# yinwoods/k8s-scheduler

Hardware: AMD Instinct MI355X
Metric: pod-node evaluations/sec (higher is better)
Workload: dtype f64

## Files before the change

k8s-scheduler_amd/csrc/ksched_commit.h:

```cpp
#pragma once

#include <hip/hip_runtime.h>

#include <type_traits>

#ifndef KSCHED_XCHG_DEBUG
#define KSCHED_XCHG_DEBUG 0
#endif
#ifndef KSCHED_COMMIT_SPLIT
#define KSCHED_COMMIT_SPLIT 0
#endif

#include "ksched_pipe.h"

namespace ksched {

namespace {

constexpr int kSpcHashBits = 11;
constexpr int kSpcHash = 1 << kSpcHashBits;
template <bool LAG3>
constexpr int spc_slots() { return LAG3 ? 192 : 128; }
static_assert(spc_slots<true>() + 1 <= kRescueMaxT, "RescueReq::ti must hold the persistent commit's touched slots");
constexpr int kSpcInvalid = kSpcHash - 1;
constexpr int kGS = 14;
constexpr int kFoldMaskBytes = 16;

constexpr uint64_t kSkipKeyBits = 0x7ff8000000000badull;
__device__ __forceinline__ double skip_key() { return __longlong_as_double((long long)kSkipKeyBits); }
__device__ __forceinline__ float screen_y(int64_t a, double y) {
    return (a > 0 && a < (1ll << 52)) ? (float)y : __builtin_nanf("");
}

struct alignas(16) TouchY {
    float c, m, p, w;
};
__device__ __forceinline__ TouchY touch_stage(int64_t a0, int64_t a1, int64_t a2, double y0, double y1, double y2) {
    return TouchY{screen_y(a0, y0), screen_y(a1, y1), screen_y(a2, y2), 0.0f};
}
__device__ __forceinline__ bool touch_need(float qc, float qm, float qp, float thr, const TouchY &ty, int64_t rc, int64_t rm,
                                           int64_t rp, int64_t n0, int64_t n1, int64_t n2, bool active, float *v) {
    bool lo;
    *v = screen_pair(qc, qm, qp, ty.c, ty.m, ty.p, n0 >= rc, n1 >= rm, n2 >= rp, &lo);
    return active && !(*v < thr);
}
template <int PRIO, int DOM, bool F53>
__device__ __forceinline__ bool touch_column(float qc, float qm, float qp, float thr, const TouchY &ty, bool active,
// ... 435 lines not shown
        if (SCR)
            thr0 = (wave == 0 && pj) ? (int32_t)(uint32_t)(load_i64<COH>(
                                           reinterpret_cast<const int64_t *>(A.lists + (size_t)lane * K + 1) + 6) >> 32) : 0;
#pragma unroll
        for (int u = 0; u < kHeadPer; ++u) {
            const int e = tid + u * kSpcThreads;
            w0[u] = 0; w1[u] = 0;
            if (e < 64 * K && e / K < nb) {
                const uint64_t *w = reinterpret_cast<const uint64_t *>(A.lists + e);
                if (COH) { w0[u] = ld_coh(w); w1[u] = ld_coh(w + 1); }
                else { w0[u] = w[0]; w1[u] = w[1]; }
            }
        }
    };
    if constexpr (!COH) load_lists();

    int n1 = 0, n2 = 0, nin = 0;
    uint64_t dbg_x1 = 0;
    (void)dbg_x1;
    const double rcf = (double)rc, rmf = (double)rm, rpf = (double)rp;
    const double y3 = recip(3.0);
    double *Srow = m.S + (size_t)lane * kSpcRow;
    uint64_t smv[3] = {0, 0, 0};
    auto key_inherited = [&](int ne, auto sl) {
        int dfl = 0;
        double pk = -__builtin_inf();
        int32_t pi = kNoIdx, ps = -1;
        const float thrf = SCR ? m.thr[lane] : 0.0f;
        const float qc = screen_req(rc), qm = screen_req(rm), qp = screen_req(rp);
        int64_t nex = 0;
        int tv = 0;
        if constexpr (SCR) {
            const int ev = wave + lane * kSpcWaves;
            tv = ev < ne ? sl(ev) : 0;
        }
        for (int e = wave, u = 0; e < ne; e += kSpcWaves, ++u) {
            const int t = SCR ? __builtin_amdgcn_readlane(tv, u) : sl(e);
            const SpcSlot &x = m.T[t];
            const int64_t *x0 = m.s0 + e * 3;
            const bool f0 = fits(rc, rm, rp, sel, x0[0], x0[1], x0[2], x.labels, LAB);
            const bool f1 = fits(rc, rm, rp, sel, x.cur[0], x.cur[1], x.cur[2], x.labels, LAB);
            dfl += (int)f1 - (int)f0;
            const double *yy = m.iy + e * 6;
            double k;
            if constexpr (SCR) {
                const bool any = touch_column<PRIO, DOM, F53>(qc, qm, qp, thrf, m.iyt[e], pj, f1, rc, rm, rp, rcf, rmf, rpf,
                                                              x.cur[0], x.cur[1], x.cur[2], yy, y3, x.price, &k);
                Srow[t] = k;
                if (!any) continue;
                ++nex;
            } else {
                ++nex;
                const bool el = pair_key_fast<PRIO, DOM, F53>(f1, rc, rm, rp, rcf, rmf, rpf, x.cur[0], x.cur[1], x.cur[2],
                                                              yy[0], yy[1], yy[2], yy[3], yy[4], yy[5], y3, x.price, &k);
                k = el ? k : -__builtin_inf();
                Srow[t] = k;
            }
            const bool up = k != -__builtin_inf() && better(k, x.idx, pk, pi);
            pk = up ? k : pk; pi = up ? x.idx : pi; ps = up ? t : ps;
        }
        if constexpr (SCR) {
            if (nex > 0 || A.fold_all) {
                m.pbk[wave * 64 + lane] = pk;
                m.pbx[wave * 64 + lane] = ((int64_t)ps << 32) | (uint32_t)pi;
                if (lane == 0) atomicOr(&m.fm[3], 1u << wave);
            }
        } else {
            m.pbk[wave * 64 + lane] = pk;
            m.pbx[wave * 64 + lane] = ((int64_t)ps << 32) | (uint32_t)pi;
        }
        if (dfl != 0) atomicAdd(&m.dfacc[lane], dfl);
        if (SCR && A.dbg && lane == 0 && wave < ne) {
            atomicAdd(reinterpret_cast<unsigned long long *>(&A.dbg[16]), (unsigned long long)((ne - 1 - wave) / kSpcWaves + 1));
            atomicAdd(reinterpret_cast<unsigned long long *>(&A.dbg[17]), (unsigned long long)nex);
        }
    };
    auto hash_lists = [&]() {
#pragma unroll
        for (int u = 0; u < kHeadPer; ++u) {
            const int e = tid + u * kSpcThreads;
            if (e < 64 * K) {
                const int j = e / K, q = e % K;
                const bool v = (uint32_t)(w1[u] >> 32) != 0;
                const double key = v ? __longlong_as_double((long long)w0[u]) : -__builtin_inf();
                const int32_t idx = v ? (int32_t)(uint32_t)w1[u] : kNoIdx;
                m.LK[q * 64 + j] = key;
                m.LI[q * 64 + j] = idx;
                m.HP[q * 64 + j] = idx == kNoIdx ? kSpcInvalid : spc_pos_insert(m.hk, idx);
            }
        }
    };
    if constexpr (!COH) {
        n1 = A.xin->count;
        XRec xi{};
        if (wave == 0 && lane < n1) xi = load_xrec<COH>(A.xin->e, lane);
        for (int w = tid; w < kSpcHash; w += kSpcThreads) m.hk[w] = -1;
// ... 144 lines not shown
                SpcSlot &x = m.T[slot];
                x.idx = xi.idx; x.mine = 0;
                for (int r = 0; r < 3; ++r) { m.s0[lane * 3 + r] = xi.sb[r]; x.sb[r] = xi.cur[r]; x.cur[r] = xi.cur[r]; }
                x.labels = xi.labels; x.price = xi.price; x.pad = 0;
                m.ti[slot] = xi.idx;
                m.gs[lane] = slot;
                if constexpr (SCR) {
                    double st[6];
                    stage_state(st, xi.cur);
#pragma unroll
                    for (int r = 0; r < 6; ++r) m.iy[lane * 6 + r] = st[r];
                    m.iyt[lane] = touch_stage(xi.cur[0], xi.cur[1], xi.cur[2], st[3], st[4], st[5]);
                } else {
                    stage_state(m.iy + lane * 6, xi.cur);
                }
                if (dup) m.x2s[slot] = -1;
                else atomicOr(&m.tkc[h >> 5], 1u << (h & 31));
            }
            if (lane == 0) m.ctl[3] = n2 + __popcll(nm);
        }
        __syncthreads();
        if (tid == 0 && A.trace_row) A.trace_row[23] = wall_clock64();
        nin = m.ctl[3];
        key_inherited(n1, [&](int e) { return (int)m.gs[e]; });
        __syncthreads();
        if (tid == 0 && A.trace_row) A.trace_row[24] = wall_clock64();
    }

    int32_t fcc = 0;
    double rbk = -__builtin_inf();
    int32_t rbi = kNoIdx, rbs = -1;
    constexpr bool RB2 = COH && PRIO == kPrioResource && DOM == kDomAll;
    bool trk = false;
    int cv = 0, cut = 0;
    int32_t my_idx = 0, my_feas = 0;
    int32_t my_src = 0;
    double my_score = 0.0;
    int32_t my_g = -2, my_q = -1, my_s = -1, my_h = kSpcInvalid;
    int nT = nin, done = nb, W = 64;
    int nresc = 0;
    int rcredit = 0, rmax = 0;
    if constexpr (COH) {
        const int c = A.loc->rescue_credit + A.rescue_rate;
        rcredit = c < 4 * A.rescue_cap ? c : 4 * A.rescue_cap;
        rmax = rcredit >= 2 * A.rescue_cap ? A.rescue_max : A.rescue_low;
    }
    int64_t placed = 0, nrounds = 0, nfail = 0, niters = 0, nseq = 0;
    int nfull = 0;
    static_assert(kSpcWaves <= 32, "SpcSmem::fm: a wave mask is one 32-bit word");
    constexpr uint32_t kAllWaves = 0xffffffffu >> (32 - kSpcWaves);
    auto fm_count = [&](int w, int64_t v) {
        if (v) atomicAdd(reinterpret_cast<unsigned long long *>(&A.dbg[w]), (unsigned long long)v);
    };
    if (wave == 0) {
        int64_t ds2 = 0;
        double xk = -__builtin_inf();
        int32_t xix = kNoIdx, xe = -1;
        if (LAG3 && A.batch >= 2 && n2 > 0 && pj) {
            ds2 = (int64_t)smv[0];
            xk = __longlong_as_double((long long)smv[1]);
            xix = (int32_t)(uint32_t)smv[2];
            xe = (int32_t)(smv[2] >> 32);
        }
        fcc = pj ? (int32_t)(fc0v + m.dfacc[lane] + ds2) : 0;
        cut = cut0;
#pragma unroll
        for (int q = 0; q < K; ++q) cv += m.LI[q * 64 + lane] != kNoIdx;
        if constexpr (SCR) {
            uint32_t wm = (uint32_t)__builtin_amdgcn_readfirstlane((int)m.fm[3]) | (A.fold_all & kAllWaves);
            if (dbg && lane == 0) {
                fm_count(34, wm == 0);
                m.ctl[3] = 0;
            }
            for (; wm != 0; wm &= wm - 1u) {
                const int w = __builtin_ctz(wm);
                const double k = m.pbk[w * 64 + lane];
                const int64_t x = m.pbx[w * 64 + lane];
                const int32_t xi = (int32_t)(uint32_t)x;
                if (k != -__builtin_inf() && better(k, xi, rbk, rbi)) { rbk = k; rbi = xi; rbs = (int32_t)(x >> 32); }
            }
        } else {
            for (int w = 0; w < kSpcWaves; ++w) {
                const double k = m.pbk[w * 64 + lane];
                const int64_t x = m.pbx[w * 64 + lane];
                const int32_t xi = (int32_t)(uint32_t)x;
                if (k != -__builtin_inf() && better(k, xi, rbk, rbi)) { rbk = k; rbi = xi; rbs = (int32_t)(x >> 32); }
            }
        }
        if (LAG3 && xix != kNoIdx) {
            if (m.x2s[xe] >= 0) {
                if (better(xk, xix, rbk, rbi)) { rbk = xk; rbi = xix; rbs = m.x2s[xe]; }
            } else {
                for (int e = 0; e < n2; ++e) {
                    if (m.x2s[e] < 0) continue;
                    const double k = Srow[m.x2s[e]];
                    const int32_t xi = m.ti[m.x2s[e]];
                    if (k != -__builtin_inf() && better(k, xi, rbk, rbi)) { rbk = k; rbi = xi; rbs = m.x2s[e]; }
                }
            }
        }
        if (lane == 0) { m.ctl[0] = 0; m.ctl[2] = 0; }
    }

    auto rekey_row = [&](int f, double &wk, int32_t &wi, int &s) {
        const int64_t fc = rl64(rc, f), fm = rl64(rm, f), fp = rl64(rp, f);
        const uint64_t fs = (uint64_t)rl64((int64_t)sel, f);
        const double fcf = (double)fc, fmf = (double)fm, fpf = (double)fp;
        double *row = m.S + (size_t)f * kSpcRow;
        int64_t nrk = 0;
        for (int t0 = 0; t0 < nT; t0 += 64) {
            const int t = t0 + lane;
            double k = -__builtin_inf();
            int32_t x = kNoIdx, ts_ = t;
            if (t < nT && row[t] != row[t]) {
                const SpcSlot &y = m.T[t];
                const bool fy = fits(fc, fm, fp, fs, y.cur[0], y.cur[1], y.cur[2], y.labels, LAB);
                k = lane_key<PRIO, DOM, LAB, F53>(fy, fc, fm, fp, fcf, fmf, fpf, y.cur[0], y.cur[1], y.cur[2], y3, y.price);
                row[t] = k;
                x = k != -__builtin_inf() ? y.idx : kNoIdx;
                ++nrk;
            }
            wave_argbest_fast(k, x, ts_);
            if (x != kNoIdx && better(k, x, wk, wi)) { wk = k; wi = x; s = ts_; }
        }
// ... 20 lines not shown
                const bool u1 = v[u + 1] != -__builtin_inf() && better(v[u + 1], x[u + 1], k1, i1);
                if constexpr (T2) { const double o1 = u1 ? k1 : v[u + 1]; q1 = o1 > q1 ? o1 : q1; }
                if (u1) { k1 = v[u + 1]; i1 = x[u + 1]; s1 = t + u + 1; }
            }
        }
        for (; t < nT; ++t) {
            const double v = Srow[t];
            const int32_t x = m.ti[t];
            const bool u0 = v != -__builtin_inf() && better(v, x, k0, i0);
            if constexpr (T2) { const double o0 = u0 ? k0 : v; q0 = o0 > q0 ? o0 : q0; }
            if (u0) { k0 = v; i0 = x; s0 = t; }
        }
        q0 = q1 > q0 ? q1 : q0;
        if (k1 != -__builtin_inf() && better(k1, i1, k0, i0)) {
            q0 = k0 > q0 ? k0 : q0;
            k0 = k1; i0 = i1; s0 = s1;
        } else {
            q0 = k1 > q0 ? k1 : q0;
        }
        rbk = k0; rbi = i0; rbs = s0;
        if constexpr (T2) m.rb2[lane] = __double2float_ru(q0);
    };
    int c = 0;
    if (COH && tid == 0 && A.trace_row) A.trace_row[25] = wall_clock64();
    uint64_t *const tr1 = (COH && tid == 0) ? A.trace_row : nullptr;
    bool first = true;
    const uint64_t t_pro = dbg ? __builtin_amdgcn_s_memtime() - t_start : 0;
    for (;;) {
        if (dbg) t_mark = __builtin_amdgcn_s_memtime();
        if (wave == 0) {
            const int cend = (c + W < nb) ? c + W : nb;
            lds_order();
            for (int w = lane * 4; w < kSpcHash; w += 256) *reinterpret_cast<int4 *>(m.own + w) = make_int4(64, 64, 64, 64);
            lds_order();
            const uint64_t fitm = __ballot(fcc != 0);
            const bool act = lane >= c && lane < cend && ((fitm >> lane) & 1);
            constexpr int G = K < 8 ? K : 8;
            const uint32_t hp_at = lds_addr(m.HP + lane), own_at = lds_addr(m.own);
            uint32_t am = 0;
#pragma unroll
            for (int g = 0; g < K; g += G) {
                int32_t hp[G], tw[G];
                lds_gather<G, 5>(hp_at + g * 256, lds_addr(m.tkc), hp, tw);
#pragma unroll
                for (int u = 0; u < G; ++u) am |= (((uint32_t)tw[u] >> (hp[u] & 31)) & 1u) ? 0u : (1u << (g + u));
            }
            if (!act) am = 0;
            const uint32_t am1 = am & (am - 1u), amr = am1 & (am1 - 1u);
            const int32_t q0 = am ? (int32_t)__builtin_ctz(am) : 0, q1 = am1 ? (int32_t)__builtin_ctz(am1) : 0;
            int32_t h0, h1;
            lds_read2(hp_at + q0 * 256, hp_at + q1 * 256, h0, h1);
            int32_t pq = -1, ph = kSpcInvalid;
            for (int it = 0;; ++it) {
                ++niters;
                int32_t nq, nh;
                {
                    int32_t o0, o1;
                    lds_read2(own_at + h0 * 4, own_at + h1 * 4, o0, o1);
                    const bool ok0 = am != 0u && o0 >= lane, ok1 = am1 != 0u && o1 >= lane;
                    nq = ok0 ? q0 : (ok1 ? q1 : -1);
                    nh = ok0 ? h0 : (ok1 ? h1 : kSpcInvalid);
                    if (__ballot(amr != 0u && !ok0 && !ok1) != 0) {
                        ++nfull;
                        nq = -1; nh = kSpcInvalid;
#pragma unroll
                        for (int g = K - G; g >= 0; g -= G) {
                            int32_t hp[G], ow[G];
                            lds_gather<G, 0>(hp_at + g * 256, own_at, hp, ow);
#pragma unroll
// ... 2 lines not shown
                                nq = ok ? g + u : nq;
                                nh = ok ? hp[u] : nh;
                            }
                        }
                    }
                }
                const bool changed = __ballot(act && nq != pq) != 0;
                if (act && pq >= 0) m.own[ph] = 64;
                lds_order();
                pq = nq; ph = nh;
                if (!changed && it > 0) break;
                if (act && pq >= 0) atomicMin(&m.own[ph], lane);
                lds_order();
            }
            const uint64_t gm = __ballot(act && pq >= 0);
            if (lane >= c && lane < cend) {
                my_g = act ? (pq >= 0 ? 0 : -1) : -2;
                my_q = pq;
                my_h = act && pq >= 0 ? ph : kSpcInvalid;
                my_s = act && pq >= 0 ? nT + lanes_below(gm) : -1;
            }
            const bool in = lane >= c && lane < cend;
            if (in && my_g == 0) my_g = m.LI[my_q * 64 + lane];
            m.gn[lane] = in ? my_g : -2;
            m.gq[lane] = my_q;
            m.gs[lane] = my_s;
            m.fcg[lane] = 0;
            if constexpr (SCR) {
                if (lane < 3) m.fm[lane] = 0;
            }
            if (lane == 0) { m.ctl[0] = c; m.ctl[1] = cend; }
        }
        __syncthreads();
        if (first && tr1) tr1[49] = wall_clock64();
        if (dbg) { const uint64_t t = __builtin_amdgcn_s_memtime(); t_s1 += t - t_mark; t_mark = t; }
        const int rc0 = m.ctl[0], rce = m.ctl[1];
        {
            double pk = -__builtin_inf();
            int32_t pi = kNoIdx, ps = -1;
            if (wave == 0 && lane >= rc0 && lane < rce && m.gn[lane] >= 0) {
                const uint64_t *src = reinterpret_cast<const uint64_t *>(A.lists + (size_t)lane * K + m.gq[lane]) + 2;
                uint64_t v[5];
#pragma unroll
                for (int w = 0; w < 5; ++w) v[w] = COH ? ld_coh(src + w) : src[w];
                const int64_t n0 = wsub((int64_t)v[0], rc), n1 = wsub((int64_t)v[1], rm), n2 = wsub((int64_t)v[2], 1);
                const double nf0 = (double)n0, nf1 = (double)n1, nf2 = (double)n2;
                uint64_t *o = m.GS + (size_t)lane * kGS;
                if constexpr (SCR) {
                    const double ny0 = recip_or_zero(n0, nf0), ny1 = recip_or_zero(n1, nf1), ny2 = recip_or_zero(n2, nf2);
                    SpcSlot &x = m.T[my_s];
                    x.idx = my_g; x.mine = 1;
                    x.sb[0] = (int64_t)v[0]; x.sb[1] = (int64_t)v[1]; x.sb[2] = (int64_t)v[2];
                    x.cur[0] = n0; x.cur[1] = n1; x.cur[2] = n2;
                    x.labels = v[3]; x.price = __uint_as_float((uint32_t)v[4]); x.pad = 0;
                    m.ti[my_s] = my_g;
                    *reinterpret_cast<TouchY *>(o) = touch_stage(n0, n1, n2, ny0, ny1, ny2);
                    o[8] = (uint64_t)__double_as_longlong(nf0); o[9] = (uint64_t)__double_as_longlong(nf1);
                    o[10] = (uint64_t)__double_as_longlong(nf2);
                    o[11] = (uint64_t)__double_as_longlong(ny0);
// ... 578 lines not shown
```

k8s-scheduler_amd/csrc/ksched_ctx.h:

```cpp
#pragma once

#include <hip/hip_runtime.h>
#include <rccl/rccl.h>

#include <algorithm>
#include <chrono>
#include <condition_variable>
#include <cstdint>
#include <memory>
#include <mutex>
#include <optional>
#include <string>
#include <vector>

#include "ksched.h"
#include "ksched_exact.h"
#include "ksched_kernels.h"
#include "ksched_pipe.h"
#include "ksched_stream.h"

struct ksched_group {
    int nranks = 0, dev = 0;
    int64_t block_bytes = 0;
    std::vector<const char *> send;
// ... 77 lines not shown
    DevBuf<int32_t> bprio, btidx, bdepth, bseg;
    DevBuf<void> vws;
    DevBuf<void> pws;
    DevBuf<uint64_t> trace;
    DevBuf<uint64_t> trace_wg;
    DevBuf<uint64_t> xdbg;
    DevBuf<int32_t> xmin;
};

struct ksched_diag {
    bool trace = false;
    std::string trace_dump;
    std::string trace_wg;
    std::string xchg_dump;
    bool commit_stamps = false;
    bool merge_stamps = false;
    bool debug = false;
    bool no_screen = false;
    bool no_pairs = false;
    bool no_seed = false;
    bool touch_screen = true;
    bool no_fold_mask = false;
    bool early_inh = true;
    bool poison = false;
    std::optional<uint32_t> lds_fill;
    int lds_role = 7;
    int lds_lo = 0;
    std::optional<int> lds_hi;
    uint32_t jitter = 0;
    bool plain_launch = false;
    int exact1_bs = 1024;
    int xchg_diag = 0;
    int64_t epoch_base = 0;
    int64_t persist_timeout_ms = 10000;
    int64_t exchange_timeout_ms = 2000;
    int rescue_max = 4;
    int rescue_rate = 4;
    int rescue_cap = 16;
    int rescue_low = 2;
    int rescue_look = 0;
};

struct ksched_ctx {
    ksched_opts o{};
    int dev = 0;
    int cus = 256;
// ... 122 lines not shown
```

k8s-scheduler_amd/csrc/ksched_diag.hip:

```cpp
#include <cstdio>
#include <cstdlib>
#include <cstring>

#include "ksched_ctx.h"

namespace ksched {

static int env_int(const char *name, int dflt) {
    const char *v = std::getenv(name);
    return v && *v ? std::atoi(v) : dflt;
}
static std::string env_str(const char *name) {
    const char *v = std::getenv(name);
    return v ? v : "";
}

void read_env(ksched_diag *d) {
    d->trace = env_int("KSCHED_PERSIST_TRACE", 0) != 0;
    d->trace_dump = env_str("KSCHED_TRACE_DUMP");
    d->trace_wg = env_str("KSCHED_TRACE_WG");
    d->xchg_dump = env_str("KSCHED_XCHG_DUMP");
    d->commit_stamps = env_int("KSCHED_COMMIT_STAMPS", 0) != 0;
    d->merge_stamps = env_int("KSCHED_MERGE_STAMPS", 0) != 0;
    d->debug = env_int("KSCHED_DEBUG", 0) != 0;
    d->no_screen = env_int("KSCHED_NO_SCREEN", 0) != 0;
    d->no_pairs = env_int("KSCHED_NO_PAIRS", 0) != 0;
    d->no_seed = env_int("KSCHED_NO_SEED", 0) != 0;
    d->touch_screen = env_int("KSCHED_NO_TOUCH_SCREEN", 0) == 0;
    d->no_fold_mask = env_int("KSCHED_NO_FOLD_MASK", 0) != 0;
    d->early_inh = env_int("KSCHED_NO_EARLY_INH", 0) == 0;
    d->poison = env_int("KSCHED_POISON", 0) != 0;
    if (const std::string f = env_str("KSCHED_LDS_FILL"); !f.empty()) d->lds_fill = (uint32_t)std::strtoul(f.c_str(), nullptr, 0);
    d->lds_role = env_int("KSCHED_LDS_ROLE", 7);
    d->lds_lo = env_int("KSCHED_LDS_LO", 0);
    if (!env_str("KSCHED_LDS_HI").empty()) d->lds_hi = env_int("KSCHED_LDS_HI", 0);
    d->jitter = (uint32_t)env_int("KSCHED_JITTER", 0);
    d->plain_launch = env_int("KSCHED_PLAIN_LAUNCH", 0) != 0;
    d->exact1_bs = env_int("KSCHED_EXACT1_BS", 1024);
    d->xchg_diag = env_int("KSCHED_XCHG_DIAG", 0);
    d->epoch_base = env_int("KSCHED_XCHG_EPOCH_BASE", 0);
    d->persist_timeout_ms = env_int("KSCHED_PERSIST_TIMEOUT_MS", 10000);
    d->exchange_timeout_ms = env_int("KSCHED_EXCHANGE_TIMEOUT_MS", 2000);
    d->rescue_max = env_int("KSCHED_RESCUE_MAX", 4);
    d->rescue_rate = env_int("KSCHED_RESCUE_RATE", 4);
    d->rescue_cap = env_int("KSCHED_RESCUE_CAP", 16);
    d->rescue_low = env_int("KSCHED_RESCUE_LOW", 2);
    d->rescue_look = env_int("KSCHED_RESCUE_LOOK", 0);
}

static void write_u64(const std::string &path, const int64_t *hdr, size_t nhdr, const std::vector<uint64_t> &t) {
    if (FILE *f = std::fopen(path.c_str(), "wb")) {
        if (nhdr) std::fwrite(hdr, 8, nhdr, f);
        std::fwrite(t.data(), 8, t.size(), f);
// ... 53 lines not shown
                    "exactly %.4f | sequential columns %lld, exactly %.4f | rescue re-keys %lld\n", (long long)hd[16],
                    (double)hd[17] / std::max<int64_t>(1, hd[16]), (long long)hd[18], (double)hd[19] / std::max<int64_t>(1, hd[18]),
                    (long long)hd[20], (double)hd[21] / std::max<int64_t>(1, hd[20]), (long long)hd[22]);
        if (hd[14])
            fprintf(stderr, "persist commit guess: iterations %lld, of them past the two lowest entries (all K scanned) %lld | "
                    "pods resolved one by one %lld\n", (long long)hd[5], (long long)hd[8], (long long)hd[31]);
        if (hd[14])
            fprintf(stderr, "persist commit: batches=%lld rounds/batch %.3f guess iterations/round %.2f failures %lld | "
                    "cycles/batch: before the wait %.0f (other waves %.0f) entry to past the wait %.0f (poll %.0f, poll + barrier %.0f, early read sufficed %.3f, early inh read sufficed %lld of %lld) | prologue %.0f guess %.0f evaluate %.0f check %.0f total %.0f\n",
                    (long long)hd[14], (double)hd[12] / hd[14], (double)hd[5] / std::max<int64_t>(1, hd[12]),
                    (long long)hd[13], (double)hd[6] / hd[14], (double)hd[9] / hd[14] / 11.0, (double)hd[7] / hd[14], (double)hd[10] / hd[14], (double)hd[11] / hd[14], (double)hd[15] / hd[14], (long long)hd[29], (long long)hd[30], (double)hd[0] / hd[14],
                    (double)hd[1] / hd[14], (double)hd[2] / hd[14], (double)hd[3] / hd[14], (double)hd[4] / hd[14]);
        if (hd[14])
            fprintf(stderr, "persist commit rescans: steps with a worsened holder %lld, every holder kept %lld | plain rescans "
                    "%lld, %.0f cycles each | with the second-best key %lld, %.0f cycles each\n", (long long)hd[23],
                    (long long)hd[24], (long long)hd[25], (double)hd[26] / std::max<int64_t>(1, hd[25]), (long long)hd[27],
                    (double)hd[28] / std::max<int64_t>(1, hd[27]));
        if (hd[14] && hd[16])
            fprintf(stderr, "persist commit fold masks: checks that read no partials %lld of %lld, partial rows read %lld | "
                    "wave-0 states that read none %lld of %lld | confirm-fold columns visited %lld skipped %lld | batches "
                    "with a check that read none after one that read some %lld\n", (long long)hd[32], (long long)hd[12],
                    (long long)hd[33], (long long)hd[34], (long long)hd[14], (long long)hd[35], (long long)hd[36],
                    (long long)hd[37]);
    }
    if (c->d->mdbg) {
        int64_t hm[8];
        if (hipMemcpy(hm, c->d->mdbg, sizeof(hm), hipMemcpyDeviceToHost) == hipSuccess && hm[7]) {
            const double nwg = (double)hm[7];
            fprintf(stderr, "persist merge: merges=%lld | cycles/merge: loads %.0f rank-heads %.0f barrier %.0f "
                    "global-heads %.0f rank-entries %.0f write %.0f\n", (long long)hm[7], hm[0] / nwg, hm[1] / nwg,
                    hm[2] / nwg, hm[3] / nwg, hm[4] / nwg, hm[5] / nwg);
        }
    }
    if (!cnt) return;
    const double us = 0.01 / (double)cnt;
    fprintf(stderr,
            "persist trace: %lld batches, period %.2f us | to-score %.2f score %.2f merge %.2f to-commit %.2f "
            "commit %.2f commit-gap %.2f (to loop top %.2f, top to past the wait %.2f) | wg0: poll %.2f apply %.2f "
            "score %.2f (rows %.2f slowest-wave %.2f fold %.2f stores %.2f) | merger poll %.2f\n",
            (long long)cnt, 0.01 * (double)(int64_t)(at(last, 4) - at(first, 4)) / (double)std::max<int64_t>(1, last - first),
            sum[0] * us, sum[1] * us, sum[2] * us, sum[3] * us, sum[4] * us, sum[5] * us, sum[14] * us, sum[15] * us, sum[6] * us, sum[7] * us,
            sum[8] * us, sum[10] * us, sum[11] * us, sum[12] * us, sum[13] * us, sum[9] * us);
    if (nscr)
        fprintf(stderr, "persist screen (WG 0 wave 0): %lld of %lld batches screened | pass 1 / seed pass %.2f us, other waves "
                "%.2f us, bound %.2f us, pass 2 / single pass %.2f us, exact phase %.2f us (%.2f of the workgroup's %d rows needed; pair lists in %lld batches, "
                "%.1f pairs each)\n", (long long)nscr, (long long)cnt,
// ... 189 lines not shown
```

k8s-scheduler_amd/csrc/ksched_engine.hip:

```cpp
#include <cmath>
#include <cstdio>
#include <cstring>

#include "ksched_ctx.h"
#include "ksched_why.h"

using namespace ksched;

namespace {

hipError_t ev_take(ksched_ctx *c, int *idx) {
    if (c->ev_used >= c->ev_pool.size()) {
        hipEvent_t e;
        hipError_t r = hipEventCreate(&e);
        if (r != hipSuccess) return r;
        c->ev_pool.push_back(e);
    }
    *idx = (int)c->ev_used++;
    return hipSuccess;
}

hipError_t ev_begin(ksched_ctx *c, bool on, int *e0, hipStream_t s) {
    if (!on) return hipSuccess;
    hipError_t r = ev_take(c, e0);
// ... 242 lines not shown
    const size_t inh_b = align_up(inh_bytes(B), 256);
    const size_t need = part_b + 4 * lists_b + 5 * xb + prog_b + resc_b + inh_b;
    if (c->d->pws.bytes < need) c->d_prog = nullptr;
    HIPCHK(c, c->d->pws.reserve(need));
    char *w = static_cast<char *>(c->d->pws.p);
    a.nodes = c->d->nodes; a.n_local = n;
    a.pods = PodArgs{c->d->rc, c->d->rm, c->d->rp, c->d->sel, c->p};
    a.ctl = reinterpret_cast<Ctl *>(c->d->cursor.p);
    a.part = reinterpret_cast<Cand *>(w);
    a.lring = w + part_b;
    a.lists_bytes = (int64_t)lists_b;
    a.xring = a.lring + 4 * lists_b;
    a.xbuf_bytes = (int64_t)xb;
    a.prog = reinterpret_cast<uint64_t *>(a.xring + 5 * xb);
    a.rescue = c->diag.rescue_max <= 0 ? nullptr : reinterpret_cast<char *>(a.prog) + prog_b;
    a.rescue_max = c->diag.rescue_max;
    a.rescue_rate = c->diag.rescue_rate;
    a.rescue_look = c->diag.rescue_look;
    a.rescue_cap = c->diag.rescue_cap;
    a.rescue_low = c->diag.rescue_low;
    a.touch_screen = c->diag.touch_screen ? 1 : 0;
    a.early_inh = c->diag.early_inh ? 1 : 0;
    a.no_fold_mask = c->diag.no_fold_mask ? 1 : 0;
    if (c->diag.jitter) a.jitter = c->diag.jitter * 2654435761u + (uint32_t)(++c->jitter_calls) * 40503u + 1u;
    a.inh = reinterpret_cast<char *>(a.prog) + prog_b + resc_b;
    c->d_prog = a.prog;
    c->prog_G = G;
    c->prog_rows = R;
    c->prog_B = B;
    a.out = OutArgs{c->d->oidx, c->d->osc, c->d->ofeas};
    fill_xchg_args(c, &a);
    a.err = c->d->err;
    a.timeout_ticks = c->diag.persist_timeout_ms * 100000;
    a.no_screen = c->diag.no_screen ? 1 : 0;
    a.no_pairs = c->diag.no_pairs ? 1 : 0;
    a.no_seed = c->diag.no_seed ? 1 : 0;
    if (c->diag.trace) {
        const int64_t cap = 4 * (c->p / B) + 64;
        HIPCHK(c, c->d->trace.reserve((size_t)cap * kTraceCols * 8));
        HIPCHK(c, hipMemsetAsync(c->d->trace, 0, c->d->trace.bytes, c->stream));
        a.trace = c->d->trace;
        a.trace_cap = c->trace_rows();
    }
    if (!c->diag.trace_wg.empty()) {
        const int64_t elems = (4 * (c->p / B) + 64) * (int64_t)G;
        HIPCHK(c, c->d->trace_wg.reserve((size_t)elems * 8));
// ... 450 lines not shown
```

k8s-scheduler_amd/csrc/ksched_kernels.h:

```cpp
#pragma once

#include "ksched_device.h"

namespace ksched {

struct alignas(16) XRec {
    int32_t idx;
    int32_t pad;
    int64_t cur[3];
    int64_t sb[3];
    uint64_t labels;
    float price;
    int32_t pad2;
    int64_t pad3;
};
static_assert(sizeof(XRec) == 80, "XRec layout");

template <bool COH>
__device__ __forceinline__ void add_i64(int64_t *p, int64_t v) {
    if (COH) st_coh(p, (uint64_t)((int64_t)ld_coh(p) + v)); else *p += v;
}

struct alignas(16) XBuf {
    int32_t count;
// ... 57 lines not shown
constexpr int kRecWords = (int)(sizeof(Rec) / 4);
constexpr int msg_words(int K) { return K * kRecWords + 2; }

struct PersistArgs;
struct PersistLocal;
struct CommitArgs {
    const Rec *lists;
    const int64_t *fc0;
    PodArgs pods;
    const int64_t *plan;
    const int64_t *plan1;
    int64_t *plan2;
    Ctl *ctl;
    int32_t B;
    const XBuf *xin;
    const XBuf *xin2;
    XBuf *xout;
    OutArgs out;
    int64_t *dbg;
    int64_t batch;
    int64_t *cursor_at;
    PersistLocal *loc;
    int32_t release;
    char *rescue;
    int32_t rescue_n;
    int32_t rescue_max;
    int32_t rescue_cap;
    int32_t rescue_low;
    int32_t rescue_look;
    int32_t rescue_rate;
    int32_t touch_screen;
    uint32_t fold_all;
    const char *inh;
    int64_t timeout_ticks;
    int32_t *err;
    uint64_t *trace_row;
    const PersistArgs *xp;
    int64_t dbg_act;
};
constexpr int kCommitDbgWords = 48;
constexpr int kSpcThreads = 512;

template <bool COH = false>
__device__ __forceinline__ void publish_committed(const CommitArgs &A) {
    if (!COH) {
        if ((threadIdx.x & 63) == 0 && A.cursor_at) st_coh(A.cursor_at, ld_coh(&A.ctl->cursor));
// ... 119 lines not shown
```

k8s-scheduler_amd/csrc/ksched_pipe.h:

```cpp
#pragma once

#include "ksched_kernels.h"

namespace ksched {

constexpr uint32_t kXRecPipe = 96;
constexpr size_t xbuf_bytes_pipe(int B) { return 16 + (size_t)2 * B * kXRecPipe; }
__device__ __forceinline__ int64_t w64(uint32_t lo, uint32_t hi) { return (int64_t)(((uint64_t)hi << 32) | lo); }

__device__ __forceinline__ bool load_xrec_pipe(const XRec *e, int i, uint32_t tag, XRec *o) {
    const __amdgpu_buffer_rsrc_t r = coh_rsrc(e);
    const uint32_t off = (uint32_t)i * kXRecPipe;
    u32x4 c[6];
#pragma unroll
    for (int k = 0; k < 6; ++k) c[k] = ld_coh16(r, off + 16u * k);
    o->idx = (int32_t)c[0].y; o->pad = 0;
    o->cur[0] = w64(c[0].z, c[0].w); o->cur[1] = w64(c[1].y, c[1].z); o->cur[2] = w64(c[1].w, c[2].y);
    o->sb[0] = w64(c[2].z, c[2].w); o->sb[1] = w64(c[3].y, c[3].z); o->sb[2] = w64(c[3].w, c[4].y);
    o->labels = (uint64_t)w64(c[4].z, c[4].w);
    o->price = __uint_as_float(c[5].y); o->pad2 = 0; o->pad3 = 0;
    return (c[0].x == tag) & (c[1].x == tag) & (c[2].x == tag) & (c[3].x == tag) & (c[4].x == tag) & (c[5].x == tag);
}

template <bool COH>
// ... 90 lines not shown
    int64_t *mdbg;
    int64_t node_offset;
    int32_t R, rank;
    uint32_t epoch0;
    int64_t xchg_stride;
    char *rx_peer[8];
    uint64_t *prog;
    char *rescue;
    int32_t poison_lds;
    uint32_t lds_fill;
    int32_t lds_fill_role;
    int32_t lds_fill_lo, lds_fill_hi;
    uint32_t jitter;
    int32_t rescue_max;
    int32_t rescue_cap;
    int32_t rescue_low;
    int32_t rescue_look;
    int32_t rescue_rate;
    int32_t touch_screen;
    char *inh;
    int32_t early_inh;
    int32_t no_seed;
    int32_t no_fold_mask;
};
constexpr size_t inh_bytes(int B) { return (size_t)4 * B * 32 + (size_t)4 * B * 64 * 8; }
constexpr int kProgWords = 6;
constexpr int kSeedWords = 2;
__host__ __device__ inline size_t prog_seed_off(int G, int B, int commit_wgs) { return (size_t)(G + B + commit_wgs) * kProgWords; }
enum : int { kProgWaitCommit = 1, kProgScan = 2, kProgArrived = 3, kProgWaitArrive = 4, kProgMerged = 5,
             kProgWaitMerged = 6, kProgCommitted = 7, kProgIdle = 8, kProgRescue = 9, kProgWaitRescue = 10,
             kProgTimedOut = 0x80 };
__device__ __forceinline__ uint32_t hw_where() {
    uint32_t xcc, hw;
    asm volatile("s_getreg_b32 %0, hwreg(HW_REG_XCC_ID)" : "=s"(xcc));
    asm volatile("s_getreg_b32 %0, hwreg(HW_REG_HW_ID)" : "=s"(hw));
    return (xcc & 0xf) << 8 | ((hw >> 13) & 7) << 4 | ((hw >> 8) & 0xf);
}
__device__ __forceinline__ void prog_at(const PersistArgs &P, int slot, int64_t b, int phase, uint64_t seen) {
    if (!P.prog) return;
    __hip_atomic_store(P.prog + kProgWords * slot, (uint64_t)b << 8 | (uint64_t)phase, __ATOMIC_RELAXED,
                       __HIP_MEMORY_SCOPE_AGENT);
    __hip_atomic_store(P.prog + kProgWords * slot + 1, (uint64_t)hw_where() << 32 | (seen & 0xffffffffull),
                       __ATOMIC_RELAXED, __HIP_MEMORY_SCOPE_AGENT);
}
__device__ __forceinline__ void prog_add(const PersistArgs &P, int slot, uint64_t scan, uint64_t busy) {
    if (!P.prog || !P.trace) return;
// ... 168 lines not shown
```

k8s-scheduler_amd/csrc/ksched_pipe.hip:

```cpp
#include <hip/hip_fp16.h>
#include <hip/hip_runtime.h>

#include <cstdio>
#include <cstdlib>

#include "ksched_commit.h"
#include "ksched_merge.h"

#ifndef KSCHED_PIPE_PART
#define KSCHED_PIPE_PART 0
#endif

namespace ksched {

namespace {

constexpr int kSW = kPipeScoreWaves;
constexpr int kMT = kPipeMergeThreads;
constexpr int kMW = kMT / 64;
constexpr int kMS = kPipeMergeSlots;
constexpr int kPU = 4;
#ifndef KSCHED_XCHG_DEBUG
#define KSCHED_XCHG_DEBUG 0
#endif
// ... 1448 lines not shown
        ca.plan = &ctl->plan[b % kPlanRing];
        ca.plan1 = &ctl->plan[(b + kPipeLag - 1) % kPlanRing];
        ca.plan2 = &ctl->plan[(b + kPipeLag) % kPlanRing];
        ca.xin = reinterpret_cast<const XBuf *>(P.xring + (size_t)(b >= 1 ? (b - 1) % 4 : 4) * P.xbuf_bytes);
        ca.xin2 = reinterpret_cast<const XBuf *>(P.xring + (size_t)(b >= 2 ? (b - 2) % 4 : 4) * P.xbuf_bytes);
        ca.xout = reinterpret_cast<XBuf *>(P.xring + (size_t)(b % 4) * P.xbuf_bytes);
        ca.out = P.out;
        ca.batch = b;
        ca.cursor_at = &ctl->cursor_at[b % kPlanRing];
        ca.dbg = P.cdbg;
        ca.trace_row = (P.trace && b < P.trace_cap) ? P.trace + b * kTraceCols : nullptr;
        ca.loc = &loc;
        ca.rescue = P.rescue;
        ca.xp = &P;
        ca.dbg_act = nact - 1;
        ca.rescue_n = P.B;
        ca.rescue_max = P.rescue_max;
        ca.rescue_rate = P.rescue_rate;
        ca.rescue_look = P.rescue_look;
        ca.rescue_cap = P.rescue_cap;
        ca.rescue_low = P.rescue_low;
        ca.touch_screen = P.touch_screen;
        ca.fold_all = P.no_fold_mask ? ~0u : 0u;
        ca.inh = P.inh;
        ca.timeout_ticks = P.timeout_ticks;
        ca.err = P.err;
        const int rc = commit_spc_batch<K, PRIO, DOM, LAB, F53, true, kPipeThreads>(ca, cs, &pre, wait_merged, handoff, inh_ready);
        if (rc == 2) return;
        if (rc == 0) {
            if (threadIdx.x == 0) atomicCAS(P.err, 0, kErrWaitMerged);
            if (threadIdx.x < 64) publish_committed_all(ctl, 1ull << 62);
            return;
        }
        __syncthreads();
        if (threadIdx.x < kCanaryBytes / 4 && canary[threadIdx.x] != (0xA5A5A5A5u ^ threadIdx.x)) {
            if (atomicCAS(P.err, 0, kErrLdsCanary) == 0 && P.prog)
                P.prog[kProgWords * cslot + 2] = (uint64_t)b << 32 | (uint64_t)threadIdx.x << 16 | (canary[threadIdx.x] & 0xffffu);
        }
        if (threadIdx.x == 0) {
            trace_at(P, b, 4);
            prog_at(P, cslot, b, kProgCommitted, 0);
        }
        if (loc.cursor >= P.pods.p) {
            if (threadIdx.x < 64) publish_committed_all(ctl, 1ull << 62);
            return;
        }
// ... 153 lines not shown
```

Baseline: 313.6 billion.

## Overlap wave 0's first guess round with inherited key scoring in persistent commit

In the persistent (coherent) commit path, wave 0 now starts the first guess/ownership round while the other waves compute inherited keys, instead of waiting behind a barrier. Wave 0's share of key scoring is spread over the remaining waves, and each wave's per-lane best is held in registers until after the barrier. The guess is redone only if the true fit mask differs from the one it assumed. This takes key scoring off the critical path before the first round, at the cost of extra control flow, an occasional wasted guess and more register pressure. The behaviour is controlled by an environment flag and is on by default.

```diff
diff --git a/k8s-scheduler_amd/csrc/ksched_commit.h b/k8s-scheduler_amd/csrc/ksched_commit.h
--- a/k8s-scheduler_amd/csrc/ksched_commit.h
+++ b/k8s-scheduler_amd/csrc/ksched_commit.h
@@ -23,6 +23,8 @@
 constexpr int spc_slots() { return LAG3 ? 192 : 128; }
 static_assert(spc_slots<true>() + 1 <= kRescueMaxT, "RescueReq::ti must hold the persistent commit's touched slots");
 constexpr int kSpcInvalid = kSpcHash - 1;
+static_assert(kSpcInvalid >= 0 && kSpcInvalid < kSpcHash && (kSpcHash & (kSpcHash - 1)) == 0,
+              "kSpcInvalid: a position inside the table, which spc_pos_insert's probe sequence skips");
 constexpr int kGS = 14;
 constexpr int kFoldMaskBytes = 16;
 
@@ -504,7 +506,13 @@
     const double y3 = recip(3.0);
     double *Srow = m.S + (size_t)lane * kSpcRow;
     uint64_t smv[3] = {0, 0, 0};
+    [[maybe_unused]] bool early_keys = false;
+    double kp_k = -__builtin_inf();
+    int64_t kp_x = 0;
+    bool kp_w = false;
     auto key_inherited = [&](int ne, auto sl) {
+        const bool defer = COH && early_keys;
+        const int kw = defer ? wave - 1 : wave, ks = defer ? kSpcWaves - 1 : kSpcWaves;
         int dfl = 0;
         double pk = -__builtin_inf();
         int32_t pi = kNoIdx, ps = -1;
@@ -513,10 +521,10 @@
         int64_t nex = 0;
         int tv = 0;
         if constexpr (SCR) {
-            const int ev = wave + lane * kSpcWaves;
+            const int ev = kw + lane * ks;
             tv = ev < ne ? sl(ev) : 0;
         }
-        for (int e = wave, u = 0; e < ne; e += kSpcWaves, ++u) {
+        for (int e = kw, u = 0; e < ne; e += ks, ++u) {
             const int t = SCR ? __builtin_amdgcn_readlane(tv, u) : sl(e);
             const SpcSlot &x = m.T[t];
             const int64_t *x0 = m.s0 + e * 3;
@@ -543,17 +551,23 @@
         }
         if constexpr (SCR) {
             if (nex > 0 || A.fold_all) {
-                m.pbk[wave * 64 + lane] = pk;
-                m.pbx[wave * 64 + lane] = ((int64_t)ps << 32) | (uint32_t)pi;
+                if (COH && defer) {
+                    kp_k = pk; kp_x = ((int64_t)ps << 32) | (uint32_t)pi; kp_w = true;
+                } else {
+                    m.pbk[wave * 64 + lane] = pk;
+                    m.pbx[wave * 64 + lane] = ((int64_t)ps << 32) | (uint32_t)pi;
+                }
                 if (lane == 0) atomicOr(&m.fm[3], 1u << wave);
             }
+        } else if (COH && defer) {
+            kp_k = pk; kp_x = ((int64_t)ps << 32) | (uint32_t)pi; kp_w = true;
         } else {
             m.pbk[wave * 64 + lane] = pk;
             m.pbx[wave * 64 + lane] = ((int64_t)ps << 32) | (uint32_t)pi;
         }
         if (dfl != 0) atomicAdd(&m.dfacc[lane], dfl);
-        if (SCR && A.dbg && lane == 0 && wave < ne) {
-            atomicAdd(reinterpret_cast<unsigned long long *>(&A.dbg[16]), (unsigned long long)((ne - 1 - wave) / kSpcWaves + 1));
+        if (SCR && A.dbg && lane == 0 && kw < ne) {
+            atomicAdd(reinterpret_cast<unsigned long long *>(&A.dbg[16]), (unsigned long long)((ne - 1 - kw) / ks + 1));
             atomicAdd(reinterpret_cast<unsigned long long *>(&A.dbg[17]), (unsigned long long)nex);
         }
     };
@@ -744,10 +758,8 @@
         __syncthreads();
         if (tid == 0 && A.trace_row) A.trace_row[23] = wall_clock64();
         nin = m.ctl[3];
-        key_inherited(n1, [&](int e) { return (int)m.gs[e]; });
-        __syncthreads();
-        if (tid == 0 && A.trace_row) A.trace_row[24] = wall_clock64();
-    }
+    }
+    [[maybe_unused]] const bool early = COH && A.early_guess != 0;
 
     int32_t fcc = 0;
     double rbk = -__builtin_inf();
@@ -774,54 +786,47 @@
     auto fm_count = [&](int w, int64_t v) {
         if (v) atomicAdd(reinterpret_cast<unsigned long long *>(&A.dbg[w]), (unsigned long long)v);
     };
-    if (wave == 0) {
-        int64_t ds2 = 0;
-        double xk = -__builtin_inf();
-        int32_t xix = kNoIdx, xe = -1;
-        if (LAG3 && A.batch >= 2 && n2 > 0 && pj) {
-            ds2 = (int64_t)smv[0];
-            xk = __longlong_as_double((long long)smv[1]);
-            xix = (int32_t)(uint32_t)smv[2];
-            xe = (int32_t)(smv[2] >> 32);
-        }
-        fcc = pj ? (int32_t)(fc0v + m.dfacc[lane] + ds2) : 0;
-        cut = cut0;
-#pragma unroll
-        for (int q = 0; q < K; ++q) cv += m.LI[q * 64 + lane] != kNoIdx;
-        if constexpr (SCR) {
-            uint32_t wm = (uint32_t)__builtin_amdgcn_readfirstlane((int)m.fm[3]) | (A.fold_all & kAllWaves);
-            if (dbg && lane == 0) {
-                fm_count(34, wm == 0);
-                m.ctl[3] = 0;
-            }
-            for (; wm != 0; wm &= wm - 1u) {
-                const int w = __builtin_ctz(wm);
-                const double k = m.pbk[w * 64 + lane];
-                const int64_t x = m.pbx[w * 64 + lane];
-                const int32_t xi = (int32_t)(uint32_t)x;
-                if (k != -__builtin_inf() && better(k, xi, rbk, rbi)) { rbk = k; rbi = xi; rbs = (int32_t)(x >> 32); }
-            }
-        } else {
+    if constexpr (!COH) {
+        if (wave == 0) {
+            fcc = pj ? (int32_t)(fc0v + m.dfacc[lane]) : 0;
+            cut = cut0;
+#pragma unroll
+            for (int q = 0; q < K; ++q) cv += m.LI[q * 64 + lane] != kNoIdx;
             for (int w = 0; w < kSpcWaves; ++w) {
                 const double k = m.pbk[w * 64 + lane];
                 const int64_t x = m.pbx[w * 64 + lane];
                 const int32_t xi = (int32_t)(uint32_t)x;
                 if (k != -__builtin_inf() && better(k, xi, rbk, rbi)) { rbk = k; rbi = xi; rbs = (int32_t)(x >> 32); }
             }
-        }
-        if (LAG3 && xix != kNoIdx) {
-            if (m.x2s[xe] >= 0) {
-                if (better(xk, xix, rbk, rbi)) { rbk = xk; rbi = xix; rbs = m.x2s[xe]; }
-            } else {
-                for (int e = 0; e < n2; ++e) {
-                    if (m.x2s[e] < 0) continue;
-                    const double k = Srow[m.x2s[e]];
-                    const int32_t xi = m.ti[m.x2s[e]];
-                    if (k != -__builtin_inf() && better(k, xi, rbk, rbi)) { rbk = k; rbi = xi; rbs = m.x2s[e]; }
-                }
-            }
-        }
-        if (lane == 0) { m.ctl[0] = 0; m.ctl[2] = 0; }
+            if (lane == 0) { m.ctl[0] = 0; m.ctl[2] = 0; }
+        }
+    } else {
+        if (wave == 0) {
+            int64_t ds2 = 0;
+            double xk = -__builtin_inf();
+            int32_t xix = kNoIdx, xe = -1;
+            if (A.batch >= 2 && n2 > 0 && pj) {
+                ds2 = (int64_t)smv[0];
+                xk = __longlong_as_double((long long)smv[1]);
+                xix = (int32_t)(uint32_t)smv[2];
+                xe = (int32_t)(smv[2] >> 32);
+            }
+            fcc = pj ? (int32_t)(fc0v + ds2) : 0;
+            cut = cut0;
+            if (xix != kNoIdx) {
+                if (m.x2s[xe] >= 0) {
+                    if (better(xk, xix, rbk, rbi)) { rbk = xk; rbi = xix; rbs = m.x2s[xe]; }
+                } else {
+                    for (int e = 0; e < n2; ++e) {
+                        if (m.x2s[e] < 0) continue;
+                        const double k = Srow[m.x2s[e]];
+                        const int32_t xi = m.ti[m.x2s[e]];
+                        if (k != -__builtin_inf() && better(k, xi, rbk, rbi)) { rbk = k; rbi = xi; rbs = m.x2s[e]; }
+                    }
+                }
+            }
+            if (lane == 0) { m.ctl[0] = 0; m.ctl[2] = 0; }
+        }
     }
 
     auto rekey_row = [&](int f, double &wk, int32_t &wi, int &s) {
@@ -888,29 +893,41 @@
         if constexpr (T2) m.rb2[lane] = __double2float_ru(q0);
     };
     int c = 0;
-    if (COH && tid == 0 && A.trace_row) A.trace_row[25] = wall_clock64();
     uint64_t *const tr1 = (COH && tid == 0) ? A.trace_row : nullptr;
     bool first = true;
     const uint64_t t_pro = dbg ? __builtin_amdgcn_s_memtime() - t_start : 0;
+    [[maybe_unused]] uint64_t fitp = 0;
     for (;;) {
         if (dbg) t_mark = __builtin_amdgcn_s_memtime();
+        [[maybe_unused]] bool g = true, st = true;
+        [[maybe_unused]] bool more = false, skip_bar = false;
+        if constexpr (COH) { g = !first || early; st = !first; }
+#pragma nounroll
+        do {
         if (wave == 0) {
             const int cend = (c + W < nb) ? c + W : nb;
+            if (!COH || g) {
             lds_order();
             for (int w = lane * 4; w < kSpcHash; w += 256) *reinterpret_cast<int4 *>(m.own + w) = make_int4(64, 64, 64, 64);
             lds_order();
             const uint64_t fitm = __ballot(fcc != 0);
+            if constexpr (COH) fitp = fitm;
             const bool act = lane >= c && lane < cend && ((fitm >> lane) & 1);
             constexpr int G = K < 8 ? K : 8;
             const uint32_t hp_at = lds_addr(m.HP + lane), own_at = lds_addr(m.own);
             uint32_t am = 0;
+            [[maybe_unused]] int cvn = 0;
 #pragma unroll
             for (int g = 0; g < K; g += G) {
                 int32_t hp[G], tw[G];
                 lds_gather<G, 5>(hp_at + g * 256, lds_addr(m.tkc), hp, tw);
 #pragma unroll
-                for (int u = 0; u < G; ++u) am |= (((uint32_t)tw[u] >> (hp[u] & 31)) & 1u) ? 0u : (1u << (g + u));
-            }
+                for (int u = 0; u < G; ++u) {
+                    am |= (((uint32_t)tw[u] >> (hp[u] & 31)) & 1u) ? 0u : (1u << (g + u));
+                    if constexpr (COH) cvn += hp[u] != kSpcInvalid;
+                }
+            }
+            if constexpr (COH) cv = cvn;
             if (!act) am = 0;
             const uint32_t am1 = am & (am - 1u), amr = am1 & (am1 - 1u);
             const int32_t q0 = am ? (int32_t)__builtin_ctz(am) : 0, q1 = am1 ? (int32_t)__builtin_ctz(am1) : 0;
@@ -959,6 +976,9 @@
             }
             const bool in = lane >= c && lane < cend;
             if (in && my_g == 0) my_g = m.LI[my_q * 64 + lane];
+            }
+            if (!COH || st) {
+            const bool in = lane >= c && lane < cend;
             m.gn[lane] = in ? my_g : -2;
             m.gq[lane] = my_q;
             m.gs[lane] = my_s;
@@ -967,11 +987,67 @@
                 if (lane < 3) m.fm[lane] = 0;
             }
             if (lane == 0) { m.ctl[0] = c; m.ctl[1] = cend; }
-        }
-        __syncthreads();
+            }
+        }
+        if constexpr (COH) {
+            more = first && !st;
+            if (more) {
+                early_keys = early;
+                kp_w = false;
+                if (wave != 0 || !early) key_inherited(n1, [&](int e) { return (int)m.gs[e]; });
+                __syncthreads();
+                if (tr1) tr1[24] = wall_clock64();
+                if (early) {
+                    bool anyp = true;
+                    if constexpr (SCR) anyp = ((uint32_t)m.fm[3] | A.fold_all) != 0;
+                    if (kp_w) {
+                        m.pbk[wave * 64 + lane] = kp_k;
+                        m.pbx[wave * 64 + lane] = kp_x;
+                    }
+                    if (anyp) __syncthreads();
+                }
+                if (wave == 0) {
+                    fcc = pj ? fcc + m.dfacc[lane] : 0;
+                    if constexpr (SCR) {
+                        uint32_t wm = (uint32_t)__builtin_amdgcn_readfirstlane((int)m.fm[3]) |
+                                      (A.fold_all & kAllWaves & (early ? ~1u : ~0u));
+                        if (dbg && lane == 0) {
+                            fm_count(34, wm == 0);
+                            m.ctl[3] = 0;
+                        }
+                        for (; wm != 0; wm &= wm - 1u) {
+                            const int w = __builtin_ctz(wm);
+                            const double k = m.pbk[w * 64 + lane];
+                            const int64_t x = m.pbx[w * 64 + lane];
+                            const int32_t xi = (int32_t)(uint32_t)x;
+                            if (k != -__builtin_inf() && better(k, xi, rbk, rbi)) { rbk = k; rbi = xi; rbs = (int32_t)(x >> 32); }
+                        }
+                    } else {
+                        for (int w = early ? 1 : 0; w < kSpcWaves; ++w) {
+                            const double k = m.pbk[w * 64 + lane];
+                            const int64_t x = m.pbx[w * 64 + lane];
+                            const int32_t xi = (int32_t)(uint32_t)x;
+                            if (k != -__builtin_inf() && better(k, xi, rbk, rbi)) { rbk = k; rbi = xi; rbs = (int32_t)(x >> 32); }
+                        }
+                    }
+                    g = true;
+                    if (early) {
+                        g = __ballot(fcc != 0) != fitp;
+                        if (g) { niters = 0; nfull = 0; }
+                        if (dbg && lane == 0) { fm_count(38, 1); fm_count(39, g ? 1 : 0); }
+                    }
+                }
+                if (tr1) tr1[25] = wall_clock64();
+                st = true;
+            } else {
+                skip_bar = first && early;
+            }
+        }
+        } while (COH && more);
+        if (!skip_bar) __syncthreads();
         if (first && tr1) tr1[49] = wall_clock64();
         if (dbg) { const uint64_t t = __builtin_amdgcn_s_memtime(); t_s1 += t - t_mark; t_mark = t; }
-        const int rc0 = m.ctl[0], rce = m.ctl[1];
+        const int rc0 = skip_bar ? 0 : m.ctl[0], rce = skip_bar ? nb : m.ctl[1];
         {
             double pk = -__builtin_inf();
             int32_t pi = kNoIdx, ps = -1;
diff --git a/k8s-scheduler_amd/csrc/ksched_ctx.h b/k8s-scheduler_amd/csrc/ksched_ctx.h
--- a/k8s-scheduler_amd/csrc/ksched_ctx.h
+++ b/k8s-scheduler_amd/csrc/ksched_ctx.h
@@ -123,6 +123,7 @@
     bool touch_screen = true;
     bool no_fold_mask = false;
     bool early_inh = true;
+    bool early_guess = true;
     bool poison = false;
     std::optional<uint32_t> lds_fill;
     int lds_role = 7;
diff --git a/k8s-scheduler_amd/csrc/ksched_diag.hip b/k8s-scheduler_amd/csrc/ksched_diag.hip
--- a/k8s-scheduler_amd/csrc/ksched_diag.hip
+++ b/k8s-scheduler_amd/csrc/ksched_diag.hip
@@ -29,6 +29,7 @@
     d->touch_screen = env_int("KSCHED_NO_TOUCH_SCREEN", 0) == 0;
     d->no_fold_mask = env_int("KSCHED_NO_FOLD_MASK", 0) != 0;
     d->early_inh = env_int("KSCHED_NO_EARLY_INH", 0) == 0;
+    d->early_guess = env_int("KSCHED_NO_EARLY_GUESS", 0) == 0;
     d->poison = env_int("KSCHED_POISON", 0) != 0;
     if (const std::string f = env_str("KSCHED_LDS_FILL"); !f.empty()) d->lds_fill = (uint32_t)std::strtoul(f.c_str(), nullptr, 0);
     d->lds_role = env_int("KSCHED_LDS_ROLE", 7);
@@ -128,6 +129,9 @@
                     "with a check that read none after one that read some %lld\n", (long long)hd[32], (long long)hd[12],
                     (long long)hd[33], (long long)hd[34], (long long)hd[14], (long long)hd[35], (long long)hd[36],
                     (long long)hd[37]);
+        if (hd[14])
+            fprintf(stderr, "persist commit early guess: batches that guessed beside the keys %lld of %lld, guesses redone with "
+                    "the true fit mask %lld\n", (long long)hd[38], (long long)hd[14], (long long)hd[39]);
     }
     if (c->d->mdbg) {
         int64_t hm[8];
diff --git a/k8s-scheduler_amd/csrc/ksched_engine.hip b/k8s-scheduler_amd/csrc/ksched_engine.hip
--- a/k8s-scheduler_amd/csrc/ksched_engine.hip
+++ b/k8s-scheduler_amd/csrc/ksched_engine.hip
@@ -288,6 +288,7 @@
     a.touch_screen = c->diag.touch_screen ? 1 : 0;
     a.early_inh = c->diag.early_inh ? 1 : 0;
     a.no_fold_mask = c->diag.no_fold_mask ? 1 : 0;
+    a.no_early_guess = c->diag.early_guess ? 0 : 1;
     if (c->diag.jitter) a.jitter = c->diag.jitter * 2654435761u + (uint32_t)(++c->jitter_calls) * 40503u + 1u;
     a.inh = reinterpret_cast<char *>(a.prog) + prog_b + resc_b;
     c->d_prog = a.prog;
diff --git a/k8s-scheduler_amd/csrc/ksched_kernels.h b/k8s-scheduler_amd/csrc/ksched_kernels.h
--- a/k8s-scheduler_amd/csrc/ksched_kernels.h
+++ b/k8s-scheduler_amd/csrc/ksched_kernels.h
@@ -103,6 +103,7 @@
     int64_t *cursor_at;
     PersistLocal *loc;
     int32_t release;
+    int32_t early_guess;
     char *rescue;
     int32_t rescue_n;
     int32_t rescue_max;
diff --git a/k8s-scheduler_amd/csrc/ksched_pipe.h b/k8s-scheduler_amd/csrc/ksched_pipe.h
--- a/k8s-scheduler_amd/csrc/ksched_pipe.h
+++ b/k8s-scheduler_amd/csrc/ksched_pipe.h
@@ -136,6 +136,7 @@
     int32_t early_inh;
     int32_t no_seed;
     int32_t no_fold_mask;
+    int32_t no_early_guess;
 };
 constexpr size_t inh_bytes(int B) { return (size_t)4 * B * 32 + (size_t)4 * B * 64 * 8; }
 constexpr int kProgWords = 6;
diff --git a/k8s-scheduler_amd/csrc/ksched_pipe.hip b/k8s-scheduler_amd/csrc/ksched_pipe.hip
--- a/k8s-scheduler_amd/csrc/ksched_pipe.hip
+++ b/k8s-scheduler_amd/csrc/ksched_pipe.hip
@@ -1494,6 +1494,7 @@
         ca.rescue_low = P.rescue_low;
         ca.touch_screen = P.touch_screen;
         ca.fold_all = P.no_fold_mask ? ~0u : 0u;
+        ca.early_guess = P.no_early_guess ? 0 : 1;
         ca.inh = P.inh;
         ca.timeout_ticks = P.timeout_ticks;
         ca.err = P.err;
```

Result: no change. 312.4 billion (-0.4%).
